# hoadainhan66ac/celestia-app

Measured on AMD Instinct MI355X. Metric: EDS+DAH squares/sec (k=128), higher is better.
Workload: dtype u8/u32; 1 GPU; config 4: 1024 independent k=128 squares per step split over 1 GPU(s), 1024 per GPU (rank g: squares [1024g, 1024g+1024)); k=128, distinct_squares=1024, parallelism=dp1 (independent squares), layout=inplace

## Files before the change

celestia-app_amd/csrc/cda_kernels.h:

```cpp
#pragma once
#include <hip/hip_runtime.h>
#include <stdint.h>

#include "push_order.h"

namespace cda {

constexpr uint32_t kNoCopy = 0xFFFFFFFFu;

struct RsSeg {
    uint32_t n_cw;
    uint32_t src_off, src_cw, src_sh;
    uint32_t dst_off, dst_cw, dst_sh;
    uint32_t cpy_off = kNoCopy, cpy_cw = 0, cpy_sh = 0;
};
struct RsJob {
    const uint8_t* src;
    uint8_t* dst;
    uint64_t src_sq, dst_sq;
    RsSeg seg[2];
    uint32_t n_seg;
    uint32_t* err_init = nullptr;
    uint32_t prio = 0;
};
// ... 22 lines not shown

struct CellGrid {
    const uint8_t* base;
    uint64_t sq;
    uint32_t rows, cols, row_stride;
    uint32_t row0, col0, k;
};

hipError_t launch_leaves(const CellGrid& g, uint32_t n_squares, uint8_t* slots, uint32_t* err, bool check_rows,
                         bool check_cols, hipStream_t stream);
hipError_t launch_row_order(const CellGrid& g, uint32_t n_squares, uint32_t* err, hipStream_t stream);

struct Forest {
    const uint8_t* in;
    uint64_t in_sq;
    uint32_t n_trees, tree_stride, node_stride;
    uint8_t* out;
    uint64_t out_sq;
    uint8_t* roots;
    uint64_t roots_sq;
    uint8_t* root_slots;
    uint64_t rslot_sq;
    uint32_t root0;
    Forest from_square(uint64_t i0) const {
        Forest f = *this;
        f.in += i0 * in_sq;
        if (roots) f.roots += i0 * roots_sq;
        if (root_slots) f.root_slots += i0 * rslot_sq;
        return f;
    }
};
hipError_t launch_level(const Forest* f, uint32_t n_forest, uint32_t n_in, uint32_t n_squares, hipStream_t stream);
hipError_t launch_subtrees(const Forest* f, uint32_t n_forest, uint32_t n_in, uint32_t top, uint32_t n_squares,
                           hipStream_t stream);
bool pair_sha_enabled();
hipError_t launch_tree_top(const Forest* f, uint32_t n_forest, uint32_t n_in, uint32_t n_squares, uint32_t* dig,
                           uint32_t n_items, hipStream_t stream, uint32_t* n_dig_out = nullptr, bool wide = false);
hipError_t launch_data_root(const uint8_t* root_slots, uint32_t n_items, uint32_t n_squares, uint8_t* data_roots,
                            hipStream_t stream);
hipError_t launch_data_root_slots(const uint8_t* root_slots, uint32_t n_items, uint32_t n_squares,
                                  uint32_t* digests, uint8_t* data_roots, hipStream_t stream,
                                  const uint32_t* err = nullptr, int32_t* status = nullptr);
hipError_t launch_rfc_leaves(const uint8_t* slots, uint32_t n, uint32_t* digests, hipStream_t stream);
hipError_t launch_data_root_digests(const uint32_t* digests, uint32_t n_items, uint32_t n_squares,
                                    uint8_t* data_roots, hipStream_t stream, const uint32_t* err = nullptr,
                                    int32_t* status = nullptr);
hipError_t launch_slots_to_roots(const uint8_t* slots, uint32_t n_slots, uint8_t* rows, uint8_t* cols, uint32_t w,
                                 hipStream_t stream);
hipError_t launch_status(const uint32_t* err, uint32_t n_squares, int32_t* status, hipStream_t stream);

}
```

celestia-app_amd/csrc/engine.h:

```cpp
#pragma once
#include "knobs.h"
#include <hip/hip_runtime.h>
#include <stdint.h>

#include <functional>
#include <mutex>
#include <string>
#include <vector>

#include "cda_kernels.h"
#include "hash_plan.h"
#include "square_plan.h"

struct cda_share_proof_batch;
struct cda_share_proofs_out;
struct cda_namespace_plan_t;
struct cda_namespace_proofs_out;
struct cda_namespace_proof_batch;
struct cda_befp_batch;
namespace cda {
class OutRegions;
struct ResidentView;
struct SegmentEmit;
}
// ... 207 lines not shown
                   uint8_t* shares, uint8_t* nmt_nodes);
    int befp_verify(const cda_befp_batch* b, uint8_t* verdict, uint8_t* rebuilt_roots);

    enum Stage { kStageRsQ0 = 0, kStageRsQ3, kStageOrder, kStageLeaves, kStageLevels, kStageDataRoot, kNumStages };
    void set_profiling(bool on) { profiling_ = on; }
    int collect_stage_times(double* ms, uint32_t* counts, int n);

    uint32_t dev_err_n_ = 0;
    int32_t po_axis = -1;
    uint32_t po_index = 0, po_pos = 0;

  private:
    int check(hipError_t e, const char* what);
    int ensure(DevBuf& b, size_t n, const char* what) { return check(b.ensure(n), what); }
    int h2d(void* dst, const void* src, size_t n, hipStream_t s, const char* what) {
        return check(hipMemcpyAsync(dst, src, n, hipMemcpyHostToDevice, s), what);
    }
    int d2h(void* dst, const void* src, size_t n, hipStream_t s, const char* what) {
        return check(hipMemcpyAsync(dst, src, n, hipMemcpyDeviceToHost, s), what);
    }
    int fill(void* p, int v, size_t n, hipStream_t s, const char* what) {
        return check(hipMemsetAsync(p, v, n, s), what);
    }
    int launched(const char* what) { return check(hipGetLastError(), what); }
    int sync(hipStream_t s, const char* what = "hipStreamSynchronize") { return check(hipStreamSynchronize(s), what); }
    int regions_out(const OutRegions& out, const uint8_t* scratch, bool one_copy, hipStream_t s, const char* what);
    static constexpr size_t kMaxPending = 48;
    std::vector<const char*> pending_;
    bool sync_check_ = false;
    void note_stage(const char* what);
    std::string pending_stages() const;
    int run_forests(Forest* f, uint32_t n_forest, uint32_t n_in, uint32_t n, uint8_t* bufA, uint8_t* bufB,
                    uint64_t buf_sq, const uint64_t* out_off, hipStream_t s, uint32_t stop = 1,
                    bool subtrees = false);
    int subtree_min_ = 8;
    uint64_t subtree_lanes_ = 0;
    uint32_t rs16_prio_max_ = 4;
    bool rs8_prio_ = true;
    uint32_t top_fuse_nodes(uint32_t W, uint32_t n, bool* wide = nullptr) const;
    int top_fuse_ = -1;
    int top_wide_ = 2;
    int check_width(uint32_t k);
    int fail_push_order(const uint8_t* last_ns, const uint8_t* pushed_ns);
    int push_order_error(const uint32_t* err_words, uint32_t n, const uint8_t* host_q0_src, uint32_t k,
                         bool src_is_eds);
    int read_push_order(const void* d_words, uint32_t n, uint32_t* words, hipStream_t s);
    std::string fault_;

    struct Mark {
        int stage;
        hipEvent_t a, b;
    };
    void mark_begin(int stage, hipStream_t s);
    void mark_end(hipStream_t s);
    bool profiling_ = false;
    std::vector<Mark> marks_;
    std::vector<hipEvent_t> event_pool_;
    double stage_ms_[kNumStages] = {};
    uint32_t stage_n_[kNumStages] = {};
    hipEvent_t take_event();

    int device_;
    hipStream_t stream_ = nullptr;
    hipStream_t copy_out_ = nullptr;
    hipEvent_t ev_rs_ = nullptr, ev_out_ = nullptr;
    int enqueue_parity_d2h(const uint8_t* d_eds, uint32_t k, uint32_t n, uint8_t* eds, hipStream_t from,
                           hipEvent_t ready, hipEvent_t done, int eds_mode = 0, uint8_t* d_par = nullptr);
// ... 88 lines not shown
```

celestia-app_amd/csrc/engine.hip:

```cpp
#include "knobs.h"
#include "engine.h"
#include "hash_plan.h"

#include <algorithm>
#include <cstdio>
#include <cstdlib>
#include <cstring>
#include <memory>
#include <thread>
#include <vector>

#include <emmintrin.h>

#include "../../include/cda.h"
#include "leopard_tables.h"
#include "sha256_dev.h"
#include "split_layout.h"
#include "tree_index.h"

namespace cda {

static thread_local bool tl_in_call = false;
static thread_local hipStream_t tl_call_stream = nullptr;

// ... 281 lines not shown
            }
        }
        if (m.a) event_pool_.push_back(m.a);
        if (m.b) event_pool_.push_back(m.b);
    }
    marks_.clear();
    for (int i = 0; i < n && i < kNumStages; i++) {
        if (ms) ms[i] = stage_ms_[i];
        if (counts) counts[i] = stage_n_[i];
        stage_ms_[i] = 0;
        stage_n_[i] = 0;
    }
    return CDA_OK;
}

int Engine::enqueue_extend(const uint8_t* d_ods, uint32_t k, uint32_t n, uint8_t* d_eds, hipStream_t s,
                           uint32_t* err_init) {
    CDA_TRY(check_width(k));
    const Gf16Dev t = gf16(k);
    mark_begin(kStageRsQ0, s);
    RsJob q0 = d_ods ? square_job_q0(d_ods, d_eds, k) : square_job_q0_inplace(d_eds, k);
    RsJob q3 = square_job_q3(d_eds, k);
    q0.err_init = err_init;
    q0.prio = q3.prio = (k >= 256 ? n <= rs16_prio_max_ : rs8_prio_) ? 1u : 0u;
    CDA_TRY(check(launch_rs(q0, k, n, t, s), "rs Q0"));
    mark_end(s);
    mark_begin(kStageRsQ3, s);
    CDA_TRY(check(launch_rs(q3, k, n, t, s), "rs Q3"));
    mark_end(s);
    return CDA_OK;
}

int Engine::run_forests(Forest* f, uint32_t n_forest, uint32_t n_in, uint32_t n, uint8_t* bufA, uint8_t* bufB,
                        uint64_t buf_sq, const uint64_t* out_off, hipStream_t s, uint32_t stop, bool subtrees) {
    uint8_t* out = bufA;
    uint32_t m0 = n_in;
    if (subtrees && n_forest <= 2) {
        uint32_t n_trees[2] = {0, 0};
        for (uint32_t i = 0; i < n_forest && i < 2; i++) n_trees[i] = f[i].n_trees;
        const uint64_t room = n_forest > 1 ? out_off[1] - out_off[0] : buf_sq;
        const uint32_t sub = subtree_sub(n_in, stop, n, n_trees, n_forest, room, subtree_min_, subtree_lanes_);
        const bool fits = sub != 0;
        if (fits) {
            for (uint32_t i = 0; i < n_forest; i++) {
                f[i].out = out + out_off[i];
                f[i].out_sq = buf_sq;
            }
            CDA_TRY(check(launch_subtrees(f, n_forest, n_in, sub, n, s), "nmt subtrees"));
            for (uint32_t i = 0; i < n_forest; i++) {
                f[i].in = out + out_off[i];
                f[i].in_sq = buf_sq;
                f[i].tree_stride = sub;
                f[i].node_stride = 1;
            }
            out = bufB;
            m0 = sub;
        }
    }
    for (uint32_t m = m0; m >= 2 && m > stop; m /= 2) {
        for (uint32_t i = 0; i < n_forest; i++) {
            f[i].out = out + out_off[i];
            f[i].out_sq = buf_sq;
        }
        CDA_TRY(check(launch_level(f, n_forest, m, n, s), "nmt level"));
        for (uint32_t i = 0; i < n_forest; i++) {
            f[i].in = out + out_off[i];
            f[i].in_sq = buf_sq;
            f[i].tree_stride = m / 2;
            f[i].node_stride = 1;
        }
        out = out == bufA ? bufB : bufA;
    }
    return CDA_OK;
}

int Engine::dah_prepare(uint32_t W, uint32_t n, uint32_t* d_err, hipStream_t s) {
    const uint64_t slots_sq = (uint64_t)W * W * kSlot;
    CDA_TRY(ensure(leaf_, slots_sq * n, "hipMalloc leaf slots"));
    CDA_TRY(ensure(lvl_, slots_sq * n, "hipMalloc level slots"));
    CDA_TRY(ensure(root_slots_, (size_t)n * 2 * W * kSlot, "hipMalloc root slots"));
    CDA_TRY(ensure(dig_, (size_t)n * 2 * W * 32, "hipMalloc digests"));
    return d_err ? fill(d_err, 0xFF, (size_t)n * 4, s, "hipMemsetAsync") : CDA_OK;
}

int Engine::reserve(uint32_t k, uint32_t n) {
    if (!err_words(n)) return fail(CDA_ERR_OOM, "hipMalloc err words");
    CDA_TRY(dah_prepare(2 * k, n, nullptr, stream_));
    return sync(stream_);
}

void Engine::dah_forests(uint32_t W, uint8_t* d_rows, uint8_t* d_cols, Forest (&f)[2]) {
    const uint64_t slots_sq = (uint64_t)W * W * kSlot;
    f[0] = Forest{leaf_.as<uint8_t>(), slots_sq, W, W, 1, nullptr, 0, d_rows, (uint64_t)W * kNode,
                  root_slots_.as<uint8_t>(), (uint64_t)2 * W * kSlot, 0};
    f[1] = Forest{leaf_.as<uint8_t>(), slots_sq, W, 1, W, nullptr, 0, d_cols, (uint64_t)W * kNode,
                  root_slots_.as<uint8_t>(), (uint64_t)2 * W * kSlot, W};
}

int Engine::dah_chunk(const uint8_t* d_eds, uint32_t k, uint32_t i0, uint32_t m, uint32_t stop, uint32_t* d_err,
                      const Forest (&f)[2], Forest (&post)[2], hipStream_t s, bool subtrees) {
    const uint32_t W = 2 * k;
    const uint64_t slots_sq = (uint64_t)W * W * kSlot, eds_sq = (uint64_t)W * W * kShare;
    mark_begin(kStageLeaves, s);
    const CellGrid g{d_eds + i0 * eds_sq, eds_sq, W, W, W, 0, 0, k};
    CDA_TRY(check(launch_leaves(g, m, leaf_.as<uint8_t>() + i0 * slots_sq, d_err + i0, true, true, s), "leaf hashing"));
    mark_end(s);
    Forest fc[2] = {f[0].from_square(i0), f[1].from_square(i0)};
    if (W > stop) {
        mark_begin(kStageLevels, s);
        const uint64_t off[2] = {0, slots_sq / 2};
        CDA_TRY(run_forests(fc, 2, W, m, lvl_.as<uint8_t>() + i0 * slots_sq, leaf_.as<uint8_t>() + i0 * slots_sq,
                slots_sq, off, s, stop, subtrees));
        mark_end(s);
    }
    for (int i = 0; i < 2; i++) {
        post[i] = fc[i];
        post[i].in -= i0 * fc[i].in_sq;
        post[i].roots = f[i].roots;
        post[i].root_slots = f[i].root_slots;
    }
    return CDA_OK;
}

int Engine::dah_finish(uint32_t k, uint32_t i0, uint32_t n, uint32_t from, const Forest (&fb)[2], uint8_t* d_roots,
                       uint32_t* d_err, int32_t* d_status, hipStream_t s) {
    const uint32_t W = 2 * k;
    const uint64_t slots_sq = (uint64_t)W * W * kSlot;
    Forest f[2] = {fb[0].from_square(i0), fb[1].from_square(i0)};
    uint32_t* dig = dig_.as<uint32_t>() + (size_t)i0 * 2 * W * 8;
    uint8_t* rslots = root_slots_.as<uint8_t>() + (size_t)i0 * 2 * W * kSlot;
    if (d_roots) d_roots += (size_t)i0 * 32;
    d_err += i0;
    if (d_status) d_status += i0;
    const TopChoice tc = finish_top(W, n, from, top_fuse_, top_wide_, pair_sha_enabled());
    const uint32_t top = tc.top;
    const bool wide = tc.wide;
    uint32_t n_dig = 2 * W;
    if (from > 1) {
        const uint32_t stop = top ? top : 1;
        mark_begin(kStageLevels, s);
        if (from > stop) {
            const bool in_lvl = ((__builtin_ctz(W) - __builtin_ctz(from)) & 1) != 0;
            uint8_t* a = (in_lvl ? leaf_.as<uint8_t>() : lvl_.as<uint8_t>()) + i0 * slots_sq;
            uint8_t* b = (in_lvl ? lvl_.as<uint8_t>() : leaf_.as<uint8_t>()) + i0 * slots_sq;
            const uint64_t off[2] = {0, slots_sq / 2};
// ... 576 lines not shown
```

celestia-app_amd/csrc/nmt.hip:

```cpp
#include "knobs.h"
#include <algorithm>
#include <type_traits>
#include <cstdlib>

#include "cda_kernels.h"
#include "hash_plan.h"
#include "sha256_dev.h"
#include "leaf_dev.h"

namespace cda {

namespace {

constexpr size_t SH = 512;

#ifndef CDA_LEAF_WAVES
#define CDA_LEAF_WAVES 4
#endif
#ifndef CDA_LEVEL_WAVES
#define CDA_LEVEL_WAVES 4
#endif

__device__ __forceinline__ void load_chunk(const uint4* p, uint32_t (&w)[16]) {
#pragma unroll
    for (int q = 0; q < 4; q++) {
        const uint4 v = p[q];
        w[4 * q + 0] = v.x; w[4 * q + 1] = v.y; w[4 * q + 2] = v.z; w[4 * q + 3] = v.w;
    }
}
__device__ __forceinline__ void bswap16(uint32_t (&w)[16]) {
#pragma unroll
    for (int i = 0; i < 16; i++) w[i] = bswap32(w[i]);
}

__global__ __launch_bounds__(256) void row_order_kernel(const CellGrid g, uint32_t* __restrict__ err) {
    const uint32_t cell = blockIdx.x * 256 + threadIdx.x;
    if (cell >= g.rows * g.cols) return;
    const uint32_t r = cell / g.cols, c = cell % g.cols;
    const uint32_t gr = g.row0 + r, gc = g.col0 + c;
    if (gr >= g.k || gc + 1 >= g.k || c + 1 >= g.cols) return;
    const uint8_t* E = g.base + blockIdx.y * g.sq;
    uint32_t me[8], nb[8];
    load_ns_be(E + ((size_t)r * g.row_stride + c) * SH, me);
    load_ns_be(E + ((size_t)r * g.row_stride + c + 1) * SH, nb);
    if (ns_less(nb, me)) atomicMin(err + blockIdx.y, push_order::encode(0, gr, gc + 1));
}

__device__ __forceinline__ void leaf_block(const CellGrid& g, uint8_t* __restrict__ slots, uint32_t* __restrict__ err,
                                           int check_rows, int check_cols, uint32_t bx, uint32_t by,
                                           uint32_t (*ns_lds)[8]) {
    const uint32_t cell = bx * 256 + threadIdx.x;
    if (cell >= g.rows * g.cols) return;
    leaf_cell(g, slots, err, check_rows, check_cols, by, cell / g.cols, cell % g.cols, ns_lds[threadIdx.x]);
}

__global__ __launch_bounds__(256) void leaf_pair_kernel(const CellGrid g, uint8_t* __restrict__ slots,
                                                        uint32_t* __restrict__ err, int check_rows, int check_cols,
                                                        uint32_t nbx) {
    const uint32_t bx = blockIdx.x % nbx, by = blockIdx.x / nbx;
    const uint32_t cell = bx * 128 + (threadIdx.x >> 1);
    if (cell >= g.rows * g.cols) return;
    const bool A = threadIdx.x & 1;
    const size_t sq = by;
    const uint32_t r = cell / g.cols, c = cell % g.cols;
    const uint32_t gr = g.row0 + r, gc = g.col0 + c, k = g.k;
// ... 40 lines not shown
        for (int t = 0; t < 7; t++) w[t] = body_word(tail[t], tail[t + 1]);
        w[7] = body_word(tail[7], cur[0]);
#pragma unroll
        for (int t = 8; t < 16; t++) w[t] = body_word(cur[t - 8], cur[t - 7]);
#pragma unroll
        for (int i = 0; i < 8; i++) tail[i] = cur[8 + i];
        h.compress(w, A);
    }
#pragma unroll
    for (int t = 0; t < 7; t++) w[t] = body_word(tail[t], tail[t + 1]);
    w[7] = __builtin_amdgcn_perm(tail[7], tail[7], 0x02030C0Cu) | 0x8000u;
#pragma unroll
    for (int t = 8; t < 15; t++) w[t] = 0;
    w[15] = kLeafMsgBits;
    h.compress(w, A);
    uint32_t D[8], out[kSlotWords];
    h.digest(A, D);
    leaf_node_words(nsw, D, out);
    if (!A) store_slot(slots + (sq * (size_t)g.rows * g.cols + cell) * kSlot, out);
}

__global__ __launch_bounds__(256) __attribute__((amdgpu_waves_per_eu(CDA_LEAF_WAVES))) void leaf_kernel(
    const CellGrid g, uint8_t* __restrict__ slots, uint32_t* __restrict__ err, int check_rows, int check_cols,
    uint32_t nbx, uint32_t nblocks) {
    __shared__ __attribute__((aligned(16))) uint32_t ns_lds[256][8];
    for (uint32_t b = blockIdx.x; b < nblocks; b += gridDim.x)
        leaf_block(g, slots, err, check_rows, check_cols, b % nbx, b / nbx, ns_lds);
}

struct Forest2 {
    Forest f[2];
};

template <bool MID = true>
__device__ __forceinline__ void hash_node(const uint32_t (&L)[kSlotWords], const uint32_t (&R)[kSlotWords],
                                          uint32_t (&o)[kSlotWords]) {
    uint32_t w[16];
    ShaState st;
    sha_init(st);
    if (MID && is_parity_head(L)) {
        w[14] = node_msg(L, R, 14);
        w[15] = node_msg(L, R, 15);
        sha_compress_from<kNodeParityRounds>(st, kNodeParityMid, kNodeParityHead, w);
    } else {
#pragma unroll
        for (int i = 0; i < 16; i++) w[i] = node_msg(L, R, i);
        sha_compress(st, w);
    }
#pragma unroll
    for (int b = 1; b < 3; b++) {
#pragma unroll
        for (int i = 0; i < 16; i++) w[i] = node_msg(L, R, 16 * b + i);
        sha_compress(st, w);
    }
    inner_node_words(L, R, st.h, o);
}

__device__ __forceinline__ void level_block(const Forest2& fs, uint32_t n_in, uint32_t bx, uint32_t by, uint32_t bz) {
    const Forest& F = fs.f[bz];
    const uint32_t n_out = n_in / 2;
    const uint32_t idx = bx * 256 + threadIdx.x;
    if (idx >= F.n_trees * n_out) return;
    const size_t sq = by;
    uint32_t t, p;
    if (F.node_stride == 1) {
        if (n_out >= 2) {
            const uint32_t hn = n_out / 2, per = F.n_trees * hn;
            const uint32_t h = idx / per, r = idx % per;
            t = r / hn; p = h * hn + r % hn;
        } else {
            t = idx; p = 0;
        }
    } else {
        p = idx / F.n_trees; t = idx % F.n_trees;
    }
    const uint8_t* base = F.in + sq * F.in_sq;
    const uint8_t* l = base + ((size_t)t * F.tree_stride + (size_t)(2 * p) * F.node_stride) * kSlot;
    const uint8_t* rr = l + (size_t)F.node_stride * kSlot;
    uint32_t L[kSlotWords], R[kSlotWords];
    load_slot_be(l, L);
    load_slot_be(rr, R);
    uint32_t o[kSlotWords];
    hash_node(L, R, o);
    if (n_out == 1) {
        if (F.roots) {
            uint16_t* d16 = reinterpret_cast<uint16_t*>(F.roots + sq * F.roots_sq + (size_t)t * kNode);
#pragma unroll
            for (int i = 0; i < kNode / 2; i++) d16[i] = (uint16_t)(o[i / 2] >> (16 * (i & 1)));
        }
        if (F.root_slots) store_slot(F.root_slots + sq * F.rslot_sq + (size_t)(F.root0 + t) * kSlot, o);
    } else {
        store_slot(F.out + sq * F.out_sq + ((size_t)t * n_out + p) * kSlot, o);
    }
}

__global__ __launch_bounds__(256) __attribute__((amdgpu_waves_per_eu(CDA_LEVEL_WAVES))) void level_kernel(
    const Forest2 fs, uint32_t n_in, uint32_t nbx, uint32_t nsq, uint32_t nblocks) {
    for (uint32_t b = blockIdx.x; b < nblocks; b += gridDim.x) {
        const uint32_t bx = b % nbx, r = b / nbx;
        level_block(fs, n_in, bx, r % nsq, r / nsq);
    }
}

__global__ __launch_bounds__(256) __attribute__((amdgpu_waves_per_eu(3))) void subtree_kernel(
    const Forest2 fs, uint32_t n_in, uint32_t slog, uint32_t nbx, uint32_t nsq, uint32_t nblocks) {
    const uint32_t S = 1u << slog;
    const uint32_t top = n_in >> slog;
    for (uint32_t b = blockIdx.x; b < nblocks; b += gridDim.x) {
        const uint32_t bx = b % nbx, r = b / nbx;
        const size_t sq = r % nsq;
        const Forest& F = fs.f[r / nsq];
        const uint32_t lanes = F.n_trees * top;
        const uint32_t idx = bx * 256 + threadIdx.x;
        if (idx >= lanes) continue;
        const uint32_t t = idx % F.n_trees, s = idx / F.n_trees;
        const uint8_t* in = F.in + sq * F.in_sq + ((size_t)t * F.tree_stride + (size_t)s * S * F.node_stride) * kSlot;
        const size_t leaf_step = (size_t)F.node_stride * kSlot;
        uint8_t* out = F.out + sq * F.out_sq;
        auto stack_slot = [&](uint32_t l) -> uint8_t* {
            return out + ((size_t)lanes + (size_t)(l - 1) * lanes + idx) * kSlot;
        };
        uint32_t cur[kSlotWords];
        auto load_raw = [](const uint8_t* p, uint4 (&q)[6]) {
            const uint4* v = reinterpret_cast<const uint4*>(p);
#pragma unroll
            for (int i = 0; i < 6; i++) q[i] = v[i];
        };
        auto be = [](const uint4 (&q)[6], uint32_t (&w)[kSlotWords]) {
#pragma unroll
            for (int i = 0; i < 6; i++) {
                w[4 * i] = bswap32(q[i].x); w[4 * i + 1] = bswap32(q[i].y);
                w[4 * i + 2] = bswap32(q[i].z); w[4 * i + 3] = bswap32(q[i].w);
            }
        };
        uint32_t j = 0, lvl = 0, pos = 0;
#pragma unroll 1
        for (uint32_t it = 0; it + 1 < S; it++) {
            const bool merge = it > 0 && (pos & 1);
            const uint8_t* pa = merge ? stack_slot(lvl) : in + (size_t)(2 * j) * leaf_step;
            const uint8_t* pb = merge ? pa : in + (size_t)(2 * j + 1) * leaf_step;
            uint4 a[6], b[6];
            load_raw(pa, a);
            load_raw(pb, b);
            uint32_t L[kSlotWords], R[kSlotWords];
            be(a, L);
            be(b, R);
            if (merge) {
#pragma unroll
                for (int i = 0; i < kSlotWords; i++) R[i] = bswap32(cur[i]);
            }
            const uint32_t nlvl = merge ? lvl + 1 : 1u, npos = merge ? pos >> 1 : j;
            if (!merge) j++;
            hash_node(L, R, cur);
            if (!(npos & 1) && nlvl < slog) store_slot(stack_slot(nlvl), cur);
            lvl = nlvl;
            pos = npos;
        }
        if (top == 1) {
            if (F.roots) {
                uint16_t* d16 = reinterpret_cast<uint16_t*>(F.roots + sq * F.roots_sq + (size_t)t * kNode);
#pragma unroll
                for (int i = 0; i < kNode / 2; i++) d16[i] = (uint16_t)(cur[i / 2] >> (16 * (i & 1)));
            }
            if (F.root_slots) store_slot(F.root_slots + sq * F.rslot_sq + (size_t)(F.root0 + t) * kSlot, cur);
        } else {
            store_slot(out + ((size_t)t * top + s) * kSlot, cur);
        }
    }
}

template <bool PAIR>
__device__ __forceinline__ void data_root_level(const uint32_t* __restrict__ in, uint32_t* __restrict__ out,
                                                uint32_t m) {
    const uint32_t step = PAIR ? blockDim.x / 2 : blockDim.x;
    const bool A = PAIR && (threadIdx.x & 1);
    for (uint32_t i = PAIR ? threadIdx.x / 2 : threadIdx.x; i < m; i += step) {
        uint32_t a[8], b[8], D[8];
#pragma unroll
        for (int j = 0; j < 8; j++) {
            a[j] = in[(2 * i) * 8 + j];
            b[j] = in[(2 * i + 1) * 8 + j];
        }
        rfc_inner_u<PAIR>(a, b, D, A);
        if (!A) {
#pragma unroll
            for (int j = 0; j < 8; j++) out[i * 8 + j] = D[j];
        }
    }
}


template <int R0>
__device__ __forceinline__ void pair_rounds16(uint32_t (&v)[4], const uint32_t (&kw)[16], bool A) {
    const uint32_t r1 = A ? 2u : 6u, r2 = A ? 13u : 11u, r3 = A ? 22u : 25u;
    const uint32_t mA = pair_mask();
#pragma unroll
    for (int i = 0; i < 16; i++) {
        const uint32_t S = xor3(__builtin_amdgcn_alignbit(v[0], v[0], r1), __builtin_amdgcn_alignbit(v[0], v[0], r2),
                                __builtin_amdgcn_alignbit(v[0], v[0], r3));
        const uint32_t F = pair_chmaj(v[0], v[1], v[2], mA);
// ... 433 lines not shown

hipError_t launch_leaves(const CellGrid& g, uint32_t n, uint8_t* slots, uint32_t* err, bool check_rows,
                         bool check_cols, hipStream_t s) {
    const uint64_t cells = (uint64_t)g.rows * g.cols * n;
    if (leaves_pair(cells, leaf_pair_max(), pair_sha_enabled())) {
        const uint32_t nbx2 = (g.rows * g.cols + 127) / 128;
        hipLaunchKernelGGL(leaf_pair_kernel, dim3(nbx2 * n), dim3(256), 0, s, g, slots, err, check_rows ? 1 : 0,
                           check_cols ? 1 : 0, nbx2);
        return hipGetLastError();
    }
    const uint32_t nbx = (g.rows * g.cols + 255) / 256, nblocks = nbx * n;
    if (nblocks == 0) return hipSuccess;
    hipLaunchKernelGGL(leaf_kernel, dim3(hash_grid(nblocks)), dim3(256),
                       hash_lds(reinterpret_cast<const void*>(leaf_kernel)), s, g, slots, err, check_rows ? 1 : 0,
                       check_cols ? 1 : 0, nbx, nblocks);
    return hipGetLastError();
}

hipError_t launch_level(const Forest* f, uint32_t n_forest, uint32_t n_in, uint32_t n, hipStream_t s) {
    if (n_forest < 1 || n_forest > 2 || n_in < 2) return hipErrorInvalidValue;
    Forest2 fs{};
    uint32_t maxw = 0;
    for (uint32_t i = 0; i < n_forest; i++) {
        fs.f[i] = f[i];
        maxw = maxw > f[i].n_trees * (n_in / 2) ? maxw : f[i].n_trees * (n_in / 2);
    }
    const uint32_t nbx = (maxw + 255) / 256, nblocks = nbx * n * n_forest;
    if (nblocks == 0) return hipSuccess;
    hipLaunchKernelGGL(level_kernel, dim3(hash_grid(nblocks)), dim3(256),
                       hash_lds(reinterpret_cast<const void*>(level_kernel)), s, fs, n_in, nbx, n, nblocks);
    return hipGetLastError();
}

hipError_t launch_subtrees(const Forest* f, uint32_t n_forest, uint32_t n_in, uint32_t top, uint32_t n, hipStream_t s) {
    if (n_forest < 1 || n_forest > 2 || top < 1 || n_in % top) return hipErrorInvalidValue;
    const uint32_t S = n_in / top;
    if (S < 4 || (S & (S - 1))) return hipErrorInvalidValue;
    Forest2 fs{};
    uint32_t maxw = 0;
    for (uint32_t i = 0; i < n_forest; i++) {
        fs.f[i] = f[i];
        maxw = std::max(maxw, f[i].n_trees * top);
    }
    const uint32_t nbx = (maxw + 255) / 256, nblocks = nbx * n * n_forest;
    if (nblocks == 0) return hipSuccess;
    hipLaunchKernelGGL(subtree_kernel, dim3(nblocks), dim3(256), 0, s, fs, n_in, (uint32_t)__builtin_ctz(S), nbx, n,
                       nblocks);
    return hipGetLastError();
}

bool pair_sha_enabled() {
    static const bool v = [] {
        const char* e = test_knob("CDA_TOP_PAIR");
        return !(e && atoi(e) == 0);
    }();
    return v;
}

static uint32_t data_root_mode() {
    static const bool dr_helpers = [] {
        const char* e = test_knob("CDA_DR_HELPERS");
        return !(e && atoi(e) == 0);
    }();
    return data_root_mode_for(pair_sha_enabled(), dr_helpers);
}

hipError_t launch_tree_top(const Forest* f, uint32_t n_forest, uint32_t n_in, uint32_t n, uint32_t* dig,
                           uint32_t n_items, hipStream_t s, uint32_t* n_dig_out, bool wide) {
    if (n_forest < 1 || n_forest > 2) return hipErrorInvalidValue;
    Forest2 fs{};
    uint32_t trees = 0;
    for (uint32_t i = 0; i < n_forest; i++) {
        fs.f[i] = f[i];
        trees += f[i].n_trees;
    }
    static const bool rfc_in_top = [] {
        const char* e = test_knob("CDA_TOP_RFC");
        return !(e && atoi(e) == 0);
    }();
    const TopLaunch t = tree_top_launch(n_in, n, trees, n_items, dig != nullptr, wide, pair_sha_enabled(), rfc_in_top);
// ... 67 lines not shown
```

celestia-app_amd/csrc/sha256_dev.h:

```cpp
#pragma once
#include <stdint.h>

#ifndef CDA_HD
#define CDA_HD __device__ __forceinline__
#endif

namespace cda {

constexpr int kShare = 512;
constexpr int kNs = 29;
constexpr int kNode = 90;
constexpr int kSlot = 96;
constexpr int kSlotWords = 24;

CDA_HD uint32_t rotr(uint32_t x, int n) { return __builtin_amdgcn_alignbit(x, x, n); }
__host__ __device__ constexpr uint32_t crotr(uint32_t x, int n) { return (x >> n) | (x << (32 - n)); }
CDA_HD uint32_t xor3(uint32_t a, uint32_t b, uint32_t c) { return __builtin_amdgcn_bitop3_b32(a, b, c, 0x96); }
CDA_HD uint32_t ch(uint32_t e, uint32_t f, uint32_t g) { return __builtin_amdgcn_bitop3_b32(e, f, g, 0xCA); }
CDA_HD uint32_t maj(uint32_t a, uint32_t b, uint32_t c) { return __builtin_amdgcn_bitop3_b32(a, b, c, 0xE8); }
CDA_HD uint32_t add3(uint32_t a, uint32_t b, uint32_t c) { return a + b + c; }
CDA_HD uint32_t funnel8(uint32_t hi, uint32_t lo, int s) {
    return (uint32_t)((((uint64_t)hi << 32) | lo) >> (8 * s));
}
CDA_HD uint32_t bswap32(uint32_t x) {
// ... 155 lines not shown
    for (int i = 0; i < R0; i++) w[i] = head[i];
    uint32_t a = m.v[0], b = m.v[1], c = m.v[2], d = m.v[3];
    uint32_t e = m.v[4], f = m.v[5], g = m.v[6], h = m.v[7];
    bool kc[16];
#pragma unroll
    for (int j = 0; j < 16; j++) kc[j] = j < R0;
#pragma unroll
    for (int i = R0; i < 64; i++) {
        uint32_t wi;
        if (i < 16) {
            wi = w[i];
        } else {
            const int j15 = (i - 15) & 15, j2 = (i - 2) & 15, j16 = i & 15, j7 = (i - 7) & 15;
            const uint32_t w15 = w[j15], w2 = w[j2];
            const uint32_t s0 = kc[j15] ? (crotr(w15, 7) ^ crotr(w15, 18) ^ (w15 >> 3))
                                        : xor3(rotr(w15, 7), rotr(w15, 18), w15 >> 3);
            const uint32_t s1 = kc[j2] ? (crotr(w2, 17) ^ crotr(w2, 19) ^ (w2 >> 10))
                                       : xor3(rotr(w2, 17), rotr(w2, 19), w2 >> 10);
            wi = w[j16] + s0 + w[j7] + s1;
            kc[j16] = kc[j16] && kc[j15] && kc[j7] && kc[j2];
            w[j16] = wi;
        }
        uint32_t S1 = xor3(rotr(e, 6), rotr(e, 11), rotr(e, 25));
        uint32_t t1 = add3(add3(h, S1, ch(e, f, g)), K[i], wi);
        uint32_t S0 = xor3(rotr(a, 2), rotr(a, 13), rotr(a, 22));
        uint32_t mj = maj(a, b, c);
        h = g; g = f; f = e; e = d + t1;
        d = c; c = b; b = a; a = add3(t1, S0, mj);
    }
    s.h[0] += a; s.h[1] += b; s.h[2] += c; s.h[3] += d;
    s.h[4] += e; s.h[5] += f; s.h[6] += g; s.h[7] += h;
}

CDA_HD uint32_t leaf_msg_head(const uint32_t* S, bool parity, int i) {
    if (parity) {
        if (i == 0) return 0x00FFFFFFu;
        if (i < 7) return 0xFFFFFFFFu;
        return 0xFFFF0000u | (S[0] >> 16);
    }
    if (i == 0) return S[0] >> 8;
    if (i < 7) return funnel8(S[i - 1], S[i], 1);
    return (S[6] << 24) | ((S[7] >> 24) << 16) | (S[0] >> 16);
}
CDA_HD uint32_t leaf_msg_body(uint32_t s_im8, uint32_t s_im7) { return funnel8(s_im8, s_im7, 2); }
constexpr uint32_t kLeafMsgBits = 542 * 8;

CDA_HD void leaf_node_words(const uint32_t NSW[8], const uint32_t D[8], uint32_t out[kSlotWords]) {
    uint32_t be[kSlotWords];
#pragma unroll
    for (int t = 0; t < 7; t++) be[t] = NSW[t];
    be[7] = (NSW[7] & 0xFF000000u) | (NSW[0] >> 8);
#pragma unroll
    for (int t = 8; t < 14; t++) be[t] = funnel8(NSW[t - 8], NSW[t - 7], 1);
    be[14] = (NSW[6] << 24) | ((NSW[7] >> 24) << 16) | (D[0] >> 16);
#pragma unroll
    for (int t = 15; t < 22; t++) be[t] = funnel8(D[t - 15], D[t - 14], 2);
    be[22] = D[7] << 16;
    be[23] = 0;
#pragma unroll
    for (int t = 0; t < kSlotWords; t++) out[t] = bswap32(be[t]);
}

CDA_HD uint32_t node_msg(const uint32_t* L, const uint32_t* R, int i) {
    if (i == 0) return 0x01000000u | (L[0] >> 8);
    if (i < 22) return funnel8(L[i - 1], L[i], 1);
    if (i == 22) return (funnel8(L[21], L[22], 1) & 0xFFFFFF00u) | (R[0] >> 24);
    if (i < 45) return funnel8(R[i - 23], R[i - 22], 3);
    if (i == 45) return (R[22] << 8) | 0x00800000u;
    if (i == 47) return 181u * 8u;
    return 0;
}

CDA_HD bool is_parity_min(const uint32_t* R) {
    bool all = true;
#pragma unroll
    for (int t = 0; t < 7; t++) all = all && (R[t] == 0xFFFFFFFFu);
    return all && ((R[7] >> 24) == 0xFFu);
}

CDA_HD bool is_parity_head(const uint32_t* L) {
    auto min3 = [](uint32_t a, uint32_t b, uint32_t c) { return a < b ? (a < c ? a : c) : (b < c ? b : c); };
    uint32_t m = min3(L[0], L[1], L[13] | 0xFFu);
#pragma unroll
    for (int t = 2; t < 12; t += 2) m = min3(m, L[t], L[t + 1]);
    return min3(m, L[12], L[12]) == 0xFFFFFFFFu;
}

CDA_HD void inner_node_words(const uint32_t* L, const uint32_t* R, const uint32_t D[8], uint32_t out[kSlotWords]) {
    const bool ign = is_parity_min(R);
    uint32_t be[kSlotWords];
#pragma unroll
    for (int t = 0; t < 7; t++) be[t] = L[t];
    uint32_t x7 = ign ? L[7] : R[7];
    be[7] = (L[7] & 0xFF000000u) | (x7 & 0x00FFFFFFu);
#pragma unroll
    for (int t = 8; t < 14; t++) be[t] = ign ? L[t] : R[t];
    uint32_t x14 = ign ? L[14] : R[14];
    be[14] = (x14 & 0xFFFF0000u) | (D[0] >> 16);
#pragma unroll
    for (int t = 15; t < 22; t++) be[t] = funnel8(D[t - 15], D[t - 14], 2);
    be[22] = D[7] << 16;
    be[23] = 0;
#pragma unroll
    for (int t = 0; t < kSlotWords; t++) out[t] = bswap32(be[t]);
}

CDA_HD void load_slot_be(const uint8_t* slot, uint32_t (&w)[kSlotWords]) {
    const uint4* p = reinterpret_cast<const uint4*>(slot);
#pragma unroll
    for (int q = 0; q < 6; q++) {
        const uint4 v = p[q];
        w[4 * q + 0] = bswap32(v.x); w[4 * q + 1] = bswap32(v.y);
        w[4 * q + 2] = bswap32(v.z); w[4 * q + 3] = bswap32(v.w);
    }
}
CDA_HD void store_slot(uint8_t* slot, const uint32_t (&w)[kSlotWords]) {
    uint4* p = reinterpret_cast<uint4*>(slot);
#pragma unroll
    for (int q = 0; q < 6; q++) p[q] = make_uint4(w[4 * q], w[4 * q + 1], w[4 * q + 2], w[4 * q + 3]);
}

CDA_HD uint32_t rfc_leaf_msg(const uint32_t* I, int i) {
    if (i == 0) return I[0] >> 8;
    if (i < 22) return funnel8(I[i - 1], I[i], 1);
    if (i == 22) return (funnel8(I[21], I[22], 1) & 0xFFFFFF00u) | 0x80u;
    if (i == 31) return 91u * 8u;
    return 0;
}
CDA_HD uint32_t rfc_inner_msg(const uint32_t* A, const uint32_t* B, int i) {
    if (i == 0) return 0x01000000u | (A[0] >> 8);
    if (i < 8) return funnel8(A[i - 1], A[i], 1);
    if (i == 8) return (A[7] << 24) | (B[0] >> 8);
    if (i < 16) return funnel8(B[i - 9], B[i - 8], 1);
    if (i == 16) return (B[7] << 24) | 0x00800000u;
    if (i == 31) return 65u * 8u;
    return 0;
}
// ... 199 lines not shown
```

Baseline: 22690 squares/s.

## Specialize NMT subtree hashing for parity-namespace quadrants with constant-folded SHA

Adds a parity-aware path to the NMT subtree kernel. Lanes whose subtrees lie entirely in parity namespace carry only the 8-word digest and hash with a specialized SHA routine that precomputes the constant namespace prefix and constant-folds message schedule words known to be all-ones. The non-parity path now keeps big-endian words across iterations and byte-swaps only once at the end. This cuts ALU work, register use and memory traffic for roughly three quarters of the tree lanes, at the cost of extra template instantiations and lane divergence inside a wavefront where the parity and data paths mix.

```diff
diff --git a/celestia-app_amd/csrc/cda_kernels.h b/celestia-app_amd/csrc/cda_kernels.h
--- a/celestia-app_amd/csrc/cda_kernels.h
+++ b/celestia-app_amd/csrc/cda_kernels.h
@@ -78,7 +78,7 @@
 };
 hipError_t launch_level(const Forest* f, uint32_t n_forest, uint32_t n_in, uint32_t n_squares, hipStream_t stream);
 hipError_t launch_subtrees(const Forest* f, uint32_t n_forest, uint32_t n_in, uint32_t top, uint32_t n_squares,
-                           hipStream_t stream);
+                           hipStream_t stream, uint32_t parity_k = 0);
 bool pair_sha_enabled();
 hipError_t launch_tree_top(const Forest* f, uint32_t n_forest, uint32_t n_in, uint32_t n_squares, uint32_t* dig,
                            uint32_t n_items, hipStream_t stream, uint32_t* n_dig_out = nullptr, bool wide = false);
diff --git a/celestia-app_amd/csrc/engine.h b/celestia-app_amd/csrc/engine.h
--- a/celestia-app_amd/csrc/engine.h
+++ b/celestia-app_amd/csrc/engine.h
@@ -263,7 +263,7 @@
     std::string pending_stages() const;
     int run_forests(Forest* f, uint32_t n_forest, uint32_t n_in, uint32_t n, uint8_t* bufA, uint8_t* bufB,
                     uint64_t buf_sq, const uint64_t* out_off, hipStream_t s, uint32_t stop = 1,
-                    bool subtrees = false);
+                    bool subtrees = false, uint32_t parity_k = 0);
     int subtree_min_ = 8;
     uint64_t subtree_lanes_ = 0;
     uint32_t rs16_prio_max_ = 4;
diff --git a/celestia-app_amd/csrc/engine.hip b/celestia-app_amd/csrc/engine.hip
--- a/celestia-app_amd/csrc/engine.hip
+++ b/celestia-app_amd/csrc/engine.hip
@@ -337,7 +337,8 @@
 }
 
 int Engine::run_forests(Forest* f, uint32_t n_forest, uint32_t n_in, uint32_t n, uint8_t* bufA, uint8_t* bufB,
-                        uint64_t buf_sq, const uint64_t* out_off, hipStream_t s, uint32_t stop, bool subtrees) {
+                        uint64_t buf_sq, const uint64_t* out_off, hipStream_t s, uint32_t stop, bool subtrees,
+                        uint32_t parity_k) {
     uint8_t* out = bufA;
     uint32_t m0 = n_in;
     if (subtrees && n_forest <= 2) {
@@ -351,7 +352,7 @@
                 f[i].out = out + out_off[i];
                 f[i].out_sq = buf_sq;
             }
-            CDA_TRY(check(launch_subtrees(f, n_forest, n_in, sub, n, s), "nmt subtrees"));
+            CDA_TRY(check(launch_subtrees(f, n_forest, n_in, sub, n, s, parity_k), "nmt subtrees"));
             for (uint32_t i = 0; i < n_forest; i++) {
                 f[i].in = out + out_off[i];
                 f[i].in_sq = buf_sq;
@@ -415,7 +416,7 @@
         mark_begin(kStageLevels, s);
         const uint64_t off[2] = {0, slots_sq / 2};
         CDA_TRY(run_forests(fc, 2, W, m, lvl_.as<uint8_t>() + i0 * slots_sq, leaf_.as<uint8_t>() + i0 * slots_sq,
-                slots_sq, off, s, stop, subtrees));
+                slots_sq, off, s, stop, subtrees, k));
         mark_end(s);
     }
     for (int i = 0; i < 2; i++) {
diff --git a/celestia-app_amd/csrc/nmt.hip b/celestia-app_amd/csrc/nmt.hip
--- a/celestia-app_amd/csrc/nmt.hip
+++ b/celestia-app_amd/csrc/nmt.hip
@@ -31,6 +31,14 @@
 __device__ __forceinline__ void bswap16(uint32_t (&w)[16]) {
 #pragma unroll
     for (int i = 0; i < 16; i++) w[i] = bswap32(w[i]);
+}
+__device__ __forceinline__ void load_chunk24(const uint8_t* slot, uint32_t (&w)[kSlotWords]) {
+    const uint4* p = reinterpret_cast<const uint4*>(slot);
+#pragma unroll
+    for (int q = 0; q < 6; q++) {
+        const uint4 v = p[q];
+        w[4 * q + 0] = v.x; w[4 * q + 1] = v.y; w[4 * q + 2] = v.z; w[4 * q + 3] = v.w;
+    }
 }
 
 __global__ __launch_bounds__(256) void row_order_kernel(const CellGrid g, uint32_t* __restrict__ err) {
@@ -137,7 +145,7 @@
     Forest f[2];
 };
 
-template <bool MID = true>
+template <bool MID = true, bool BE = false>
 __device__ __forceinline__ void hash_node(const uint32_t (&L)[kSlotWords], const uint32_t (&R)[kSlotWords],
                                           uint32_t (&o)[kSlotWords]) {
     uint32_t w[16];
@@ -158,7 +166,10 @@
         for (int i = 0; i < 16; i++) w[i] = node_msg(L, R, 16 * b + i);
         sha_compress(st, w);
     }
-    inner_node_words(L, R, st.h, o);
+    if (BE)
+        inner_node_be(L, R, st.h, o);
+    else
+        inner_node_words(L, R, st.h, o);
 }
 
 __device__ __forceinline__ void level_block(const Forest2& fs, uint32_t n_in, uint32_t bx, uint32_t by, uint32_t bz) {
@@ -207,70 +218,122 @@
     }
 }
 
-__global__ __launch_bounds__(256) __attribute__((amdgpu_waves_per_eu(3))) void subtree_kernel(
-    const Forest2 fs, uint32_t n_in, uint32_t slog, uint32_t nbx, uint32_t nsq, uint32_t nblocks) {
-    const uint32_t S = 1u << slog;
-    const uint32_t top = n_in >> slog;
-    for (uint32_t b = blockIdx.x; b < nblocks; b += gridDim.x) {
-        const uint32_t bx = b % nbx, r = b / nbx;
-        const size_t sq = r % nsq;
-        const Forest& F = fs.f[r / nsq];
+struct SubtreeLane {
+    uint32_t t, s;
+    bool live;
+};
+template <bool PARITY>
+__device__ __forceinline__ SubtreeLane subtree_lane(uint32_t idx, uint32_t n_trees, uint32_t top, uint32_t slog,
+                                                    uint32_t pk) {
+    if (pk == 0) return {idx % n_trees, idx / n_trees, idx < n_trees * top};
+    const uint32_t sg = max(1u, pk >> slog);
+    if (!PARITY) return {idx % pk, idx / pk, idx < pk * sg};
+    if (idx < pk * top) return {pk + idx % pk, idx / pk, true};
+    const uint32_t j = idx - pk * top;
+    return {j % pk, sg + j / pk, j < pk * (top - sg)};
+}
+
+template <bool PARITY>
+__device__ __forceinline__ void subtree_walk(const Forest& F, size_t sq, uint32_t t, uint32_t s, uint32_t slog,
+                                             uint32_t top) {
+    {
+        const uint32_t S = 1u << slog;
         const uint32_t lanes = F.n_trees * top;
-        const uint32_t idx = bx * 256 + threadIdx.x;
-        if (idx >= lanes) continue;
-        const uint32_t t = idx % F.n_trees, s = idx / F.n_trees;
+        const uint32_t idx = s * F.n_trees + t;
         const uint8_t* in = F.in + sq * F.in_sq + ((size_t)t * F.tree_stride + (size_t)s * S * F.node_stride) * kSlot;
         const size_t leaf_step = (size_t)F.node_stride * kSlot;
         uint8_t* out = F.out + sq * F.out_sq;
         auto stack_slot = [&](uint32_t l) -> uint8_t* {
             return out + ((size_t)lanes + (size_t)(l - 1) * lanes + idx) * kSlot;
         };
-        uint32_t cur[kSlotWords];
-        auto load_raw = [](const uint8_t* p, uint4 (&q)[6]) {
-            const uint4* v = reinterpret_cast<const uint4*>(p);
-#pragma unroll
-            for (int i = 0; i < 6; i++) q[i] = v[i];
-        };
-        auto be = [](const uint4 (&q)[6], uint32_t (&w)[kSlotWords]) {
-#pragma unroll
-            for (int i = 0; i < 6; i++) {
-                w[4 * i] = bswap32(q[i].x); w[4 * i + 1] = bswap32(q[i].y);
-                w[4 * i + 2] = bswap32(q[i].z); w[4 * i + 3] = bswap32(q[i].w);
-            }
-        };
+        uint32_t cur[PARITY ? 8 : kSlotWords];
         uint32_t j = 0, lvl = 0, pos = 0;
 #pragma unroll 1
         for (uint32_t it = 0; it + 1 < S; it++) {
             const bool merge = it > 0 && (pos & 1);
-            const uint8_t* pa = merge ? stack_slot(lvl) : in + (size_t)(2 * j) * leaf_step;
-            const uint8_t* pb = merge ? pa : in + (size_t)(2 * j + 1) * leaf_step;
-            uint4 a[6], b[6];
-            load_raw(pa, a);
-            load_raw(pb, b);
-            uint32_t L[kSlotWords], R[kSlotWords];
-            be(a, L);
-            be(b, R);
-            if (merge) {
-#pragma unroll
-                for (int i = 0; i < kSlotWords; i++) R[i] = bswap32(cur[i]);
+            const uint32_t nlvl = merge ? lvl + 1 : 1u, npos = merge ? pos >> 1 : j;
+            const bool push = !(npos & 1) && nlvl < slog;
+            if constexpr (PARITY) {
+                uint32_t DL[8], DR[8];
+                if (merge) {
+                    const uint4* v = reinterpret_cast<const uint4*>(stack_slot(lvl));
+                    const uint4 x = v[0], y = v[1];
+                    DL[0] = x.x; DL[1] = x.y; DL[2] = x.z; DL[3] = x.w;
+                    DL[4] = y.x; DL[5] = y.y; DL[6] = y.z; DL[7] = y.w;
+#pragma unroll
+                    for (int i = 0; i < 8; i++) DR[i] = cur[i];
+                } else {
+                    const uint4* va = reinterpret_cast<const uint4*>(in + (size_t)(2 * j) * leaf_step) + 3;
+                    const uint4* vb = reinterpret_cast<const uint4*>(in + (size_t)(2 * j + 1) * leaf_step) + 3;
+                    uint32_t ra[12], rb[12];
+#pragma unroll
+                    for (int q = 0; q < 3; q++) {
+                        const uint4 x = va[q], y = vb[q];
+                        ra[4 * q] = x.x; ra[4 * q + 1] = x.y; ra[4 * q + 2] = x.z; ra[4 * q + 3] = x.w;
+                        rb[4 * q] = y.x; rb[4 * q + 1] = y.y; rb[4 * q + 2] = y.z; rb[4 * q + 3] = y.w;
+                    }
+                    parity_slot_digest(ra, DL);
+                    parity_slot_digest(rb, DR);
+                    j++;
+                }
+                hash_parity_node(DL, DR, cur);
+                if (push) {
+                    uint4* v = reinterpret_cast<uint4*>(stack_slot(nlvl));
+                    v[0] = make_uint4(cur[0], cur[1], cur[2], cur[3]);
+                    v[1] = make_uint4(cur[4], cur[5], cur[6], cur[7]);
+                }
+            } else {
+                uint32_t L[kSlotWords], R[kSlotWords];
+                if (merge) {
+                    load_chunk24(stack_slot(lvl), L);
+#pragma unroll
+                    for (int i = 0; i < kSlotWords; i++) R[i] = cur[i];
+                } else {
+                    load_slot_be(in + (size_t)(2 * j) * leaf_step, L);
+                    load_slot_be(in + (size_t)(2 * j + 1) * leaf_step, R);
+                    j++;
+                }
+                hash_node<true, true>(L, R, cur);
+                if (push) store_slot(stack_slot(nlvl), cur);
             }
-            const uint32_t nlvl = merge ? lvl + 1 : 1u, npos = merge ? pos >> 1 : j;
-            if (!merge) j++;
-            hash_node(L, R, cur);
-            if (!(npos & 1) && nlvl < slog) store_slot(stack_slot(nlvl), cur);
             lvl = nlvl;
             pos = npos;
+        }
+        uint32_t o[kSlotWords];
+        if constexpr (PARITY) {
+            parity_slot_words(cur, o);
+        } else {
+#pragma unroll
+            for (int i = 0; i < kSlotWords; i++) o[i] = bswap32(cur[i]);
         }
         if (top == 1) {
             if (F.roots) {
                 uint16_t* d16 = reinterpret_cast<uint16_t*>(F.roots + sq * F.roots_sq + (size_t)t * kNode);
 #pragma unroll
-                for (int i = 0; i < kNode / 2; i++) d16[i] = (uint16_t)(cur[i / 2] >> (16 * (i & 1)));
+                for (int i = 0; i < kNode / 2; i++) d16[i] = (uint16_t)(o[i / 2] >> (16 * (i & 1)));
             }
-            if (F.root_slots) store_slot(F.root_slots + sq * F.rslot_sq + (size_t)(F.root0 + t) * kSlot, cur);
+            if (F.root_slots) store_slot(F.root_slots + sq * F.rslot_sq + (size_t)(F.root0 + t) * kSlot, o);
         } else {
-            store_slot(out + ((size_t)t * top + s) * kSlot, cur);
-        }
+            store_slot(out + ((size_t)t * top + s) * kSlot, o);
+        }
+    }
+}
+
+template <int FORM>
+__global__ __launch_bounds__(256) __attribute__((amdgpu_waves_per_eu(3))) void subtree_kernel(
+    const Forest2 fs, uint32_t n_in, uint32_t slog, uint32_t nbx, uint32_t nsq, uint32_t nblocks, uint32_t pk) {
+    const uint32_t top = n_in >> slog;
+    for (uint32_t b = blockIdx.x; b < nblocks; b += gridDim.x) {
+        const uint32_t bx = b % nbx, r = b / nbx;
+        const size_t sq = r % nsq;
+        const Forest& F = fs.f[r / nsq];
+        const SubtreeLane ln =
+            subtree_lane<FORM == 1>(bx * 256 + threadIdx.x, F.n_trees, top, slog, FORM == 2 ? 0u : pk);
+        if (!ln.live) continue;
+        if (FORM == 1 || (FORM == 2 && (ln.t >= pk || (ln.s << slog) >= pk)))
+            subtree_walk<true>(F, sq, ln.t, ln.s, slog, top);
+        else
+            subtree_walk<false>(F, sq, ln.t, ln.s, slog, top);
     }
 }
 
@@ -770,20 +833,49 @@
     return hipGetLastError();
 }
 
-hipError_t launch_subtrees(const Forest* f, uint32_t n_forest, uint32_t n_in, uint32_t top, uint32_t n, hipStream_t s) {
+#ifndef CDA_SUBTREE_PARITY_FORM
+#define CDA_SUBTREE_PARITY_FORM 2
+#endif
+
+hipError_t launch_subtrees(const Forest* f, uint32_t n_forest, uint32_t n_in, uint32_t top, uint32_t n, hipStream_t s,
+                           uint32_t parity_k) {
     if (n_forest < 1 || n_forest > 2 || top < 1 || n_in % top) return hipErrorInvalidValue;
     const uint32_t S = n_in / top;
     if (S < 4 || (S & (S - 1))) return hipErrorInvalidValue;
+    const uint32_t slog = (uint32_t)__builtin_ctz(S);
+    if (n == 0) return hipSuccess;
     Forest2 fs{};
     uint32_t maxw = 0;
+    bool known = CDA_SUBTREE_PARITY_FORM != 0 && parity_k >= 64 && parity_k % 64 == 0 &&
+                 !(parity_k & (parity_k - 1)) && n_in == 2 * parity_k;
     for (uint32_t i = 0; i < n_forest; i++) {
         fs.f[i] = f[i];
         maxw = std::max(maxw, f[i].n_trees * top);
-    }
+        known = known && f[i].n_trees == 2 * parity_k;
+    }
+#if CDA_SUBTREE_PARITY_FORM == 1
+    if (known) {
+        const uint32_t sg = std::max(1u, parity_k >> slog);
+        const uint32_t lanes_g = parity_k * sg, lanes_p = 2 * parity_k * top - lanes_g;
+        const uint32_t nbx_g = (lanes_g + 255) / 256, nbx_p = (lanes_p + 255) / 256;
+        hipLaunchKernelGGL(subtree_kernel<0>, dim3(nbx_g * n * n_forest), dim3(256), 0, s, fs, n_in, slog, nbx_g, n,
+                           nbx_g * n * n_forest, parity_k);
+        hipLaunchKernelGGL(subtree_kernel<1>, dim3(nbx_p * n * n_forest), dim3(256), 0, s, fs, n_in, slog, nbx_p, n,
+                           nbx_p * n * n_forest, parity_k);
+        return hipGetLastError();
+    }
+#endif
     const uint32_t nbx = (maxw + 255) / 256, nblocks = nbx * n * n_forest;
     if (nblocks == 0) return hipSuccess;
-    hipLaunchKernelGGL(subtree_kernel, dim3(nblocks), dim3(256), 0, s, fs, n_in, (uint32_t)__builtin_ctz(S), nbx, n,
-                       nblocks);
+#if CDA_SUBTREE_PARITY_FORM == 2
+    if (known) {
+        hipLaunchKernelGGL(subtree_kernel<2>, dim3(nblocks), dim3(256), 0, s, fs, n_in, slog, nbx, n, nblocks,
+                           parity_k);
+        return hipGetLastError();
+    }
+#endif
+    (void)known;
+    hipLaunchKernelGGL(subtree_kernel<0>, dim3(nblocks), dim3(256), 0, s, fs, n_in, slog, nbx, n, nblocks, 0u);
     return hipGetLastError();
 }
 
diff --git a/celestia-app_amd/csrc/sha256_dev.h b/celestia-app_amd/csrc/sha256_dev.h
--- a/celestia-app_amd/csrc/sha256_dev.h
+++ b/celestia-app_amd/csrc/sha256_dev.h
@@ -211,6 +211,41 @@
     s.h[4] += e; s.h[5] += f; s.h[6] += g; s.h[7] += h;
 }
 
+template <uint32_t KNOWN>
+CDA_HD void sha_compress_known(ShaState& s, uint32_t w[16]) {
+    constexpr uint32_t K[64] = CDA_SHA_K;
+    uint32_t a = s.h[0], b = s.h[1], c = s.h[2], d = s.h[3];
+    uint32_t e = s.h[4], f = s.h[5], g = s.h[6], h = s.h[7];
+    bool kc[16];
+#pragma unroll
+    for (int j = 0; j < 16; j++) kc[j] = (KNOWN >> j) & 1u;
+#pragma unroll
+    for (int i = 0; i < 64; i++) {
+        uint32_t wi;
+        if (i < 16) {
+            wi = w[i];
+        } else {
+            const int j15 = (i - 15) & 15, j2 = (i - 2) & 15, j16 = i & 15, j7 = (i - 7) & 15;
+            const uint32_t w15 = w[j15], w2 = w[j2];
+            const uint32_t s0 = kc[j15] ? (crotr(w15, 7) ^ crotr(w15, 18) ^ (w15 >> 3))
+                                        : xor3(rotr(w15, 7), rotr(w15, 18), w15 >> 3);
+            const uint32_t s1 = kc[j2] ? (crotr(w2, 17) ^ crotr(w2, 19) ^ (w2 >> 10))
+                                       : xor3(rotr(w2, 17), rotr(w2, 19), w2 >> 10);
+            wi = w[j16] + s0 + w[j7] + s1;
+            kc[j16] = kc[j16] && kc[j15] && kc[j7] && kc[j2];
+            w[j16] = wi;
+        }
+        uint32_t S1 = xor3(rotr(e, 6), rotr(e, 11), rotr(e, 25));
+        uint32_t t1 = add3(add3(h, S1, ch(e, f, g)), K[i], wi);
+        uint32_t S0 = xor3(rotr(a, 2), rotr(a, 13), rotr(a, 22));
+        uint32_t mj = maj(a, b, c);
+        h = g; g = f; f = e; e = d + t1;
+        d = c; c = b; b = a; a = add3(t1, S0, mj);
+    }
+    s.h[0] += a; s.h[1] += b; s.h[2] += c; s.h[3] += d;
+    s.h[4] += e; s.h[5] += f; s.h[6] += g; s.h[7] += h;
+}
+
 CDA_HD uint32_t leaf_msg_head(const uint32_t* S, bool parity, int i) {
     if (parity) {
         if (i == 0) return 0x00FFFFFFu;
@@ -265,9 +300,8 @@
     return min3(m, L[12], L[12]) == 0xFFFFFFFFu;
 }
 
-CDA_HD void inner_node_words(const uint32_t* L, const uint32_t* R, const uint32_t D[8], uint32_t out[kSlotWords]) {
+CDA_HD void inner_node_be(const uint32_t* L, const uint32_t* R, const uint32_t D[8], uint32_t be[kSlotWords]) {
     const bool ign = is_parity_min(R);
-    uint32_t be[kSlotWords];
 #pragma unroll
     for (int t = 0; t < 7; t++) be[t] = L[t];
     uint32_t x7 = ign ? L[7] : R[7];
@@ -280,8 +314,51 @@
     for (int t = 15; t < 22; t++) be[t] = funnel8(D[t - 15], D[t - 14], 2);
     be[22] = D[7] << 16;
     be[23] = 0;
+}
+CDA_HD void inner_node_words(const uint32_t* L, const uint32_t* R, const uint32_t D[8], uint32_t out[kSlotWords]) {
+    uint32_t be[kSlotWords];
+    inner_node_be(L, R, D, be);
 #pragma unroll
     for (int t = 0; t < kSlotWords; t++) out[t] = bswap32(be[t]);
+}
+
+CDA_HD void hash_parity_node(const uint32_t (&DL)[8], const uint32_t (&DR)[8], uint32_t (&D)[8]) {
+    ShaState st;
+    sha_init(st);
+    uint32_t w[16];
+    w[14] = 0xFFFFFF00u | (DL[0] >> 24);
+    w[15] = funnel8(DL[0], DL[1], 3);
+    sha_compress_from<kNodeParityRounds>(st, kNodeParityMid, kNodeParityHead, w);
+#pragma unroll
+    for (int i = 0; i < 6; i++) w[i] = funnel8(DL[i + 1], DL[i + 2], 3);
+    w[6] = (DL[7] << 8) | 0xFFu;
+#pragma unroll
+    for (int i = 7; i < 16; i++) w[i] = 0xFFFFFFFFu;
+    sha_compress_known<0xFF80u>(st, w);
+#pragma unroll
+    for (int i = 0; i < 5; i++) w[i] = 0xFFFFFFFFu;
+    w[5] = 0xFF000000u | (DR[0] >> 8);
+#pragma unroll
+    for (int i = 0; i < 7; i++) w[6 + i] = funnel8(DR[i], DR[i + 1], 1);
+    w[13] = (DR[7] << 24) | 0x00800000u;
+    w[14] = 0;
+    w[15] = 181u * 8u;
+    sha_compress_known<0xC01Fu>(st, w);
+#pragma unroll
+    for (int j = 0; j < 8; j++) D[j] = st.h[j];
+}
+CDA_HD void parity_slot_digest(const uint32_t (&r)[12], uint32_t (&D)[8]) {
+#pragma unroll
+    for (int j = 0; j < 8; j++) D[j] = __builtin_amdgcn_perm(r[3 + j], r[2 + j], 0x02030405u);
+}
+CDA_HD void parity_slot_words(const uint32_t (&D)[8], uint32_t (&out)[kSlotWords]) {
+#pragma unroll
+    for (int t = 0; t < 14; t++) out[t] = 0xFFFFFFFFu;
+    out[14] = __builtin_amdgcn_perm(D[0], D[0], 0x02030D0Du);
+#pragma unroll
+    for (int t = 15; t < 22; t++) out[t] = __builtin_amdgcn_perm(D[t - 15], D[t - 14], 0x02030405u);
+    out[22] = __builtin_amdgcn_perm(D[7], D[7], 0x0C0C0001u);
+    out[23] = 0;
 }
 
 CDA_HD void load_slot_be(const uint8_t* slot, uint32_t (&w)[kSlotWords]) {
```

After: 22800 squares/s, median of 6. No clear change (+0.5%).
